# Vidvox/hap

Hardware: AMD Instinct MI355X
Metric: RGBA GB/s + frames/sec, 8K Hap Q encode+decode (higher is better)
Workload: dtype u8; 1 GPU; C4: 7680x4320 0x1, 24 chunks, Snappy, 60-frame stream, device-resident; fragment_index=True, parallelism=single GPU

## Files before the change

hap_amd/csrc/bc_encode.hip:

```cpp
#include <hip/hip_runtime.h>
#include <stdint.h>

#include "bc_encode_core.hpp"
#include "hapgpu_runtime.hpp"

namespace {

using namespace hapbc;

template <int FMT, bool WIDE>
__device__ __forceinline__ void encode_block(const uint8_t *__restrict__ rgba, size_t row_bytes, unsigned blocks_x,
                                             uint8_t *__restrict__ out, uint8_t *__restrict__ out2 = nullptr)
{
    const unsigned by = blockIdx.y, bx = blockIdx.x * 64u + threadIdx.x;
    if (bx >= blocks_x)
        return;
    const size_t id = (size_t)by * blocks_x + bx;
    const uint8_t *src = rgba + (size_t)(4u * by) * row_bytes + 16u * bx;
    unsigned p[16];
#pragma unroll
    for (int r = 0; r < 4; r++) {
        if (WIDE) {
            const uint4 v = *reinterpret_cast<const uint4 *>(src + (size_t)r * row_bytes);
            p[4 * r + 0] = v.x; p[4 * r + 1] = v.y; p[4 * r + 2] = v.z; p[4 * r + 3] = v.w;
        } else {
            const unsigned *q = reinterpret_cast<const unsigned *>(src + (size_t)r * row_bytes);
            p[4 * r + 0] = q[0]; p[4 * r + 1] = q[1]; p[4 * r + 2] = q[2]; p[4 * r + 3] = q[3];
        }
    }
    if (FMT == kFmtRGTC1 || FMT == kFmtDXT1) {
        const uint4 b = block_of<FMT>(p);
        *reinterpret_cast<uint2 *>(out + id * 8u) = make_uint2(b.x, b.y);
    } else {
        *reinterpret_cast<uint4 *>(out + id * 16u) = block_of<FMT == kFmtYCoCgAlpha ? kFmtYCoCg : FMT>(p);
        if (FMT == kFmtYCoCgAlpha) {
            const uint4 a = block_of<kFmtRGTC1>(p);
            *reinterpret_cast<uint2 *>(out2 + id * 8u) = make_uint2(a.x, a.y);
        }
    }
}

template <int FMT, bool WIDE>
__global__ __launch_bounds__(64) void bc_encode_kernel(HapGpuPictureTable t, size_t row_bytes, unsigned blocks_x)
{
    const uint8_t *rgba = (const uint8_t *)picture_address(t, 0);
    uint8_t *out = (uint8_t *)picture_address(t, 1);
    uint8_t *out2 = FMT == kFmtYCoCgAlpha ? (uint8_t *)picture_address(t, 2) : nullptr;
    if (!rgba || !out || (FMT == kFmtYCoCgAlpha && !out2))
        return;
    encode_block<FMT, WIDE>(rgba, row_bytes, blocks_x, out, out2);
}

template <int FMT>
void launch(const HapGpuPictureTable &t, unsigned pictures, size_t row_bytes, unsigned bx, unsigned by, bool wide,
            hipStream_t stream)
{
    const dim3 grid((bx + 63u) / 64u, by, pictures), block(64);
    if (wide)
        hipLaunchKernelGGL((bc_encode_kernel<FMT, true>), grid, block, 0, stream, t, row_bytes, bx);
    else
        hipLaunchKernelGGL((bc_encode_kernel<FMT, false>), grid, block, 0, stream, t, row_bytes, bx);
}

}

extern "C" int hapgpu_k_block_encode(hapgpu_rt *rt, const HapGpuPictureTable *table, unsigned pictures, unsigned width,
                                     unsigned height, size_t row_bytes, unsigned format, int with_alpha, int wide,
                                     unsigned picture_kind)
{
    scoped_timing st(rt, 0);
    const hipStream_t stream = hapgpu_rt_stream(rt);
    const bool half = picture_kind == HAPGPU_PICTURE_RGBA16F, plane = picture_kind == HAPGPU_PICTURE_A8;
    if (picture_kind > HAPGPU_PICTURE_A8 || half != (format == 0x8E8F || format == 0x8E8E) ||
        (plane && (format != 0x8DBB || with_alpha || height / 4u > 65535u)))
        return 1;
    if (!table || !(table->column[0] || table->one[0]) || !(table->column[1] || table->one[1]) ||
        (with_alpha && (format != 0x01 || !(table->column[2] || table->one[2]))) || pictures == 0 || pictures > 65535u ||
        width == 0 || height == 0 || (width & 3u) || (height & 3u) || row_bytes < (size_t)width * HAPGPU_PICTURE_TEXEL_BYTES(picture_kind) ||
        (row_bytes & (half ? 15u : 3u)))
        return 1;
    const HapGpuPictureTable &t = *table;
    const unsigned bx = width / 4u, by = height / 4u;
    switch (format) {
    case 0x83F0: launch<kFmtDXT1>(t, pictures, row_bytes, bx, by, wide != 0, stream); break;
    case 0x83F3: launch<kFmtDXT5>(t, pictures, row_bytes, bx, by, wide != 0, stream); break;
    case 0x01:
        if (with_alpha)
            launch<kFmtYCoCgAlpha>(t, pictures, row_bytes, bx, by, wide != 0, stream);
        else
            launch<kFmtYCoCg>(t, pictures, row_bytes, bx, by, wide != 0, stream);
        break;
    case 0x8DBB:
        if (plane)
            hapgpu_launch_alpha_encode(t, pictures, bx, by, row_bytes, wide != 0, stream);
        else
            launch<kFmtRGTC1>(t, pictures, row_bytes, bx, by, wide != 0, stream);
        break;
    case 0x8E8C: hapgpu_launch_bptc_encode(t, pictures, bx, by, row_bytes, wide != 0, stream); break;
    case 0x8E8F:
    case 0x8E8E: hapgpu_launch_bc6h_encode(t, pictures, format == 0x8E8E, bx, by, row_bytes, stream); break;
    default: return 1;
    }
    return hipGetLastError() == hipSuccess ? 0 : 4;
}
```

hap_amd/csrc/bc_encode_core.hpp:

```cpp
#pragma once
#include <hip/hip_runtime.h>
#include <stdint.h>

namespace hapbc {

constexpr int kFmtDXT1 = 0, kFmtDXT5 = 1, kFmtYCoCg = 2, kFmtRGTC1 = 3;
constexpr int kFmtYCoCgAlpha = 4;

__device__ __forceinline__ int mad24(int a, int b, int c)
{
    int r;
    asm("v_mad_i32_i24 %0, %1, %2, %3" : "=v"(r) : "v"(a), "v"(b), "v"(c));
    return r;
}
template <int K>
__device__ __forceinline__ int mad24k(int a, int c)
{
    int r;
    asm("v_mad_i32_i24 %0, %1, %2, %3" : "=v"(r) : "v"(a), "i"(K), "v"(c));
    return r;
}

__device__ __forceinline__ int quant5(int v) { int t = mad24k<31>(v, 128); return (t + (t >> 8)) >> 8; }
__device__ __forceinline__ int quant6(int v) { int t = mad24k<63>(v, 128); return (t + (t >> 8)) >> 8; }
__device__ __forceinline__ int expand5(int q) { return (q << 3) | (q >> 2); }
__device__ __forceinline__ int expand6(int q) { return (q << 2) | (q >> 4); }


__device__ __forceinline__ unsigned ramp_codes(unsigned w)
{
    return w ^ (~((w >> 1) | (w >> 2)) & 0x249249u);
}

__device__ __forceinline__ uint2 alpha_block(const int (&a)[16])
{
    int lo = a[0], hi = a[0];
#pragma unroll
    for (int i = 1; i < 16; i++) {
        lo = min(lo, a[i]);
        hi = max(hi, a[i]);
    }
    const int a0 = hi, a1 = lo;
    unsigned lo24 = 0, hi24 = 0;
    if (a0 != a1) {
        const int d = a0 - a1;
        unsigned q = (unsigned)(524288.0f * __builtin_amdgcn_rcpf((float)d));
        const int rem = 524288 - (int)__umul24(q, (unsigned)d);
        q += (rem >= d ? 1u : 0u) - (rem < 0 ? 1u : 0u);
        const unsigned m = q + 1u;
        const int neg_m14 = -(int)(14u * m);
        const int start = mad24(a0, (int)(14u * m), (int)__umul24((unsigned)max(d - 6, 0), m)) + (1 << 20);
#pragma unroll
        for (int i = 0; i < 16; i++) {
            const unsigned r1 = (unsigned)mad24(a[i], neg_m14, start) >> 20;
            if (i < 8)
                lo24 = __builtin_amdgcn_alignbit(r1, lo24, 3);
            else
                hi24 = __builtin_amdgcn_alignbit(r1, hi24, 3);
        }
        lo24 = ramp_codes(lo24 >> 8);
        hi24 = ramp_codes(hi24 >> 8);
    }
    const unsigned long long bits = (unsigned long long)lo24 | ((unsigned long long)hi24 << 24);
    const unsigned long long v = (unsigned long long)(unsigned)a0 | ((unsigned long long)(unsigned)a1 << 8) | (bits << 16);
    return make_uint2((unsigned)v, (unsigned)(v >> 32));
}

struct projection {
    unsigned adir;
    unsigned flip;
    int start;
    int top;
    unsigned m24;
};

__device__ __forceinline__ unsigned index_scale(unsigned len2)
{
    unsigned m = (unsigned)(50331648.0f * __builtin_amdgcn_rcpf((float)len2));
    const int rem = (int)(50331648u - m * len2);
    m += (rem >= (int)len2 ? 1u : 0u) - (rem < 0 ? 1u : 0u);
    return m;
}

template <int CHANNELS = 3>
__device__ __forceinline__ projection make_projection(unsigned p0, unsigned p1)
{
    projection pr;
    int dir[CHANNELS];
    unsigned adir = 0, flip = 0;
    int neg = 0, base = 0;
#pragma unroll
    for (int c = 0; c < CHANNELS; c++) {
        const int a = (int)((p0 >> (8 * c)) & 255u), b = (int)((p1 >> (8 * c)) & 255u);
        dir[c] = a - b;
        const int ad = abs(dir[c]);
        adir |= (unsigned)ad << (8 * c);
        flip |= (dir[c] < 0 ? 0xFFu : 0u) << (8 * c);
        neg += dir[c] < 0 ? ad : 0;
        base = mad24(b, dir[c], base);
    }
    const unsigned len2 = __builtin_amdgcn_udot4(adir, adir, 0u, false);
    const unsigned sixth = __umulhi(len2, 0xAAAAAAABu) >> 2;
    pr.adir = adir;
    pr.flip = flip;
    pr.start = (int)sixth - base - 255 * neg;
    pr.top = (int)(len2 + sixth);
    pr.m24 = index_scale(len2);
    return pr;
}

template <bool FLIPPED = false>
__device__ __forceinline__ unsigned project4(const unsigned (&px)[16], const projection &pr)
{
    unsigned pos2 = 0;
#pragma unroll
    for (int i = 0; i < 16; i++) {
        const unsigned q = FLIPPED ? px[i] : px[i] ^ pr.flip;
        const int t = (int)__builtin_amdgcn_udot4(q, pr.adir, (unsigned)pr.start, false);
        const int pos = min(max(__mul24(t, (int)pr.m24) >> 24, 0), 3);
        pos2 = __builtin_amdgcn_alignbit((unsigned)pos, pos2, 2);
    }
    const unsigned hi = pos2 & 0xAAAAAAAAu;
    const unsigned idx = (hi ^ ((pos2 << 1) & 0xAAAAAAAAu)) | ((~hi >> 1) & 0x55555555u);
    return idx;
}

__device__ __forceinline__ unsigned pack3(int a, int b, int c) { return (unsigned)a | ((unsigned)b << 8) | ((unsigned)c << 16); }

__device__ __forceinline__ unsigned expand_565(unsigned c, bool blue)
{
    return pack3(expand5(c >> 11), expand6((c >> 5) & 63), blue ? expand5(c & 31) : 0);
}

__device__ __forceinline__ uint2 colour_block(const unsigned (&px)[16])
{
    int lo[3] = {255, 255, 255}, hi[3] = {0, 0, 0};
#pragma unroll
    for (int i = 0; i < 16; i++) {
#pragma unroll
        for (int c = 0; c < 3; c++) {
            const int v = (int)((px[i] >> (8 * c)) & 255u);
            lo[c] = min(lo[c], v);
            hi[c] = max(hi[c], v);
        }
    }
    int cov_rg = 0, cov_bg = 0;
    const int mr = lo[0] + hi[0], mg = lo[1] + hi[1], mb = lo[2] + hi[2];
#pragma unroll
    for (int i = 0; i < 16; i++) {
        const int dr = 2 * (int)(px[i] & 255u) - mr;
        const int dg = 2 * (int)((px[i] >> 8) & 255u) - mg;
        const int db = 2 * (int)((px[i] >> 16) & 255u) - mb;
        cov_rg = mad24(dr, dg, cov_rg);
        cov_bg = mad24(db, dg, cov_bg);
    }
#pragma unroll
    for (int c = 0; c < 3; c++) {
        const int inset = (hi[c] - lo[c]) >> 4;
        lo[c] += inset;
        hi[c] -= inset;
    }
    const int ar = cov_rg < 0 ? lo[0] : hi[0], br = cov_rg < 0 ? hi[0] : lo[0];
    const int ab = cov_bg < 0 ? lo[2] : hi[2], bb = cov_bg < 0 ? hi[2] : lo[2];
    const unsigned qa = (unsigned)(quant5(ar) << 11 | quant6(hi[1]) << 5 | quant5(ab));
    const unsigned qb = (unsigned)(quant5(br) << 11 | quant6(lo[1]) << 5 | quant5(bb));
    const unsigned c0 = max(qa, qb), c1 = min(qa, qb);
    unsigned idx = 0;
    if (c0 != c1)
        idx = project4(px, make_projection(expand_565(c0, true), expand_565(c1, true)));
    return make_uint2(c0 | (c1 << 16), idx);
}

typedef unsigned short pk_u16 __attribute__((ext_vector_type(2)));
typedef short pk_i16 __attribute__((ext_vector_type(2)));

__device__ __forceinline__ uint2 ycocg_colour_block(const unsigned (&cc)[16])
{
    pk_u16 lo = __builtin_bit_cast(pk_u16, cc[0]), hi = lo;
#pragma unroll
    for (int i = 1; i < 16; i++) {
        const pk_u16 v = __builtin_bit_cast(pk_u16, cc[i]);
        lo = __builtin_elementwise_min(lo, v);
        hi = __builtin_elementwise_max(hi, v);
    }
    int lo_o = lo.x, hi_o = hi.x, lo_g = lo.y, hi_g = hi.y;
    const int m = max(max(128 - lo_o, hi_o - 128), max(128 - lo_g, hi_g - 128));
    const int s = m <= 31 ? 4 : (m <= 63 ? 2 : 1);
    int prod = 0;
    pk_u16 sums = {0, 0};
#pragma unroll
    for (int i = 0; i < 16; i++) {
        int r;
        asm("v_mad_i32_i16 %0, %1, %1, %2 op_sel:[0,1,0,0]" : "=v"(r) : "v"(cc[i]), "v"(prod));
        prod = r;
        sums += __builtin_bit_cast(pk_u16, cc[i]);
    }
    const int mo = lo_o + hi_o, mg = lo_g + hi_g;
    const int cov = 4 * prod - 2 * mg * (int)sums.x - 2 * mo * (int)sums.y + 16 * mo * mg;
    lo_o = (lo_o - 128) * s + 128; hi_o = (hi_o - 128) * s + 128;
    lo_g = (lo_g - 128) * s + 128; hi_g = (hi_g - 128) * s + 128;
    int ins = (hi_o - lo_o) >> 4; lo_o += ins; hi_o -= ins;
    ins = (hi_g - lo_g) >> 4; lo_g += ins; hi_g -= ins;
    const int ag = cov < 0 ? lo_g : hi_g, bg = cov < 0 ? hi_g : lo_g;
    const int qo_a = quant5(hi_o), qo_b = quant5(lo_o), qg_a = quant6(ag), qg_b = quant6(bg);
    const unsigned qa = (unsigned)(qo_a << 11 | qg_a << 5 | (s - 1));
    const unsigned qb = (unsigned)(qo_b << 11 | qg_b << 5 | (s - 1));
    const unsigned c0 = max(qa, qb), c1 = min(qa, qb);
    unsigned idx = 0;
    if (c0 != c1) {
        const bool sw = qa < qb;
        const int eo_a = expand5(qo_a), eo_b = expand5(qo_b), eg_a = expand6(qg_a), eg_b = expand6(qg_b);
        const int d_o = sw ? eo_b - eo_a : eo_a - eo_b, d_g = sw ? eg_b - eg_a : eg_a - eg_b;
        const int p1_o = sw ? eo_a : eo_b, p1_g = sw ? eg_a : eg_b;
        const unsigned len2 = (unsigned)mad24(d_o, d_o, __mul24(d_g, d_g));
        const int sixth = (int)(__umulhi(len2, 0xAAAAAAABu) >> 2);
        const unsigned m24 = index_scale(len2);
        const int centre = 128 - 128 * s;
        const int K = mad24(d_o, centre - p1_o, mad24(d_g, centre - p1_g, sixth));
        const pk_i16 dir2 = {(short)d_o, (short)d_g};
        constexpr int kDotOffset = 1 << 17;
        const unsigned sm = (unsigned)s * m24;
        const unsigned Km = (unsigned)(K - s * kDotOffset) * m24;
        unsigned pos2 = 0;
#pragma unroll
        for (int i = 0; i < 16; i++) {
            unsigned dot;
            asm("v_dot2_i32_i16 %0, %1, %2, %3\n\ts_nop 2" : "=v"(dot) : "v"(cc[i]), "v"(__builtin_bit_cast(unsigned, dir2)), "s"(kDotOffset));
            const int pos = min(max((int)(__umul24(dot, sm) + Km) >> 24, 0), 3);
            pos2 = __builtin_amdgcn_alignbit((unsigned)pos, pos2, 2);
        }
        const unsigned hi = pos2 & 0xAAAAAAAAu;
        idx = (hi ^ ((pos2 << 1) & 0xAAAAAAAAu)) | ((~hi >> 1) & 0x55555555u);
    }
    return make_uint2(c0 | (c1 << 16), idx);
}

template <int FMT>
__device__ __forceinline__ uint4 block_of(const unsigned (&p)[16])
{
    if (FMT == kFmtRGTC1) {
        int a[16];
#pragma unroll
        for (int i = 0; i < 16; i++)
            a[i] = (int)(p[i] >> 24);
        const uint2 ab = alpha_block(a);
        return make_uint4(ab.x, ab.y, 0u, 0u);
    } else if (FMT == kFmtDXT1) {
        unsigned px[16];
#pragma unroll
        for (int i = 0; i < 16; i++)
            px[i] = p[i] & 0x00FFFFFFu;
        const uint2 cb = colour_block(px);
        return make_uint4(cb.x, cb.y, 0u, 0u);
    } else if (FMT == kFmtDXT5) {
        int a[16];
        unsigned px[16];
#pragma unroll
        for (int i = 0; i < 16; i++) {
            a[i] = (int)(p[i] >> 24);
            px[i] = p[i] & 0x00FFFFFFu;
        }
        const uint2 ab = alpha_block(a), cb = colour_block(px);
        return make_uint4(ab.x, ab.y, cb.x, cb.y);
    } else {
        int y[16];
        unsigned cc[16];
#pragma unroll
        for (int i = 0; i < 16; i++) {
            const unsigned q = p[i];
            y[i] = (int)(__builtin_amdgcn_udot4(q, 0x00010201u, 2u, false) >> 2);
            const unsigned co2 = __builtin_amdgcn_udot4(q ^ 0x00FF0000u, 0x00010001u, 2u, false);
            const unsigned cg4 = __builtin_amdgcn_udot4(q ^ 0x00FF00FFu, 0x00010201u, 4u, false);
            const pk_u16 raw = __builtin_bit_cast(pk_u16, co2 | (cg4 << 16)), sh = {1, 2};
            cc[i] = __builtin_bit_cast(unsigned, (pk_u16)(raw >> sh));
        }
        const uint2 ab = alpha_block(y), cb = ycocg_colour_block(cc);
        return make_uint4(ab.x, ab.y, cb.x, cb.y);
    }
}

}
```

hap_amd/csrc/snappy_compress_blocks.hip:

```cpp
#include <hip/hip_runtime.h>
#include <stdint.h>
#include "hapgpu_runtime.hpp"
#include "measurement_guard.h"
#include "bc_encode_core.hpp"

namespace {

constexpr unsigned kFragBytes = 8192u;
constexpr unsigned kSteps = kFragBytes / 1024u;
constexpr unsigned kTableBits = 9u;
constexpr unsigned kDistances = 4u;

template <unsigned LAYOUT> struct unit_layout;
template <> struct unit_layout<4u> {
    static constexpr unsigned block = 16u, code = 4u;
    static constexpr unsigned small32 = 0x11111111u;
    static constexpr unsigned big32 = 0x22222222u;
    static constexpr unsigned four32 = 0xCCCCCCCCu;
    static constexpr unsigned run3_12 = 0xBBBBBBBBu;
    static constexpr unsigned run15_61 = 0x22222222u;
    __device__ static constexpr unsigned fo(unsigned k) { return k == 0u ? 0u : k == 1u ? 2u : k == 2u ? 8u : 12u; }
    __device__ static constexpr unsigned fs(unsigned k) { return k == 0u ? 2u : k == 1u ? 6u : 4u; }
    __device__ static constexpr unsigned cls(unsigned k) { return k == 1u ? 1u : k == 3u ? 3u : 0u; }
};
template <> struct unit_layout<2u> {
    static constexpr unsigned block = 8u, code = 10u;
    static constexpr unsigned small32 = 0u, big32 = 0u, four32 = 0xFFFFFFFFu, run3_12 = 0xFFFFFFFFu, run15_61 = 0u;
    __device__ static constexpr unsigned fo(unsigned k) { return 4u * k; }
    __device__ static constexpr unsigned fs(unsigned) { return 4u; }
    __device__ static constexpr unsigned cls(unsigned k) { return (k & 1u) ? 1u : 0u; }
};
template <> struct unit_layout<8u> {
    static constexpr unsigned block = 16u, code = 12u;
    static constexpr unsigned small32 = 0u, big32 = 0u, four32 = 0xFFFFFFFFu, run3_12 = 0xFFFFFFFFu, run15_61 = 0u;
    __device__ static constexpr unsigned fo(unsigned k) { return 4u * k; }
    __device__ static constexpr unsigned fs(unsigned) { return 4u; }
    __device__ static constexpr unsigned cls(unsigned k) { return k == 1u ? 1u : k == 3u ? 3u : 0u; }
};
template <> struct unit_layout<6u> {
    static constexpr unsigned block = 8u, code = 2u;
    static constexpr unsigned small32 = 0x55555555u, big32 = 0xAAAAAAAAu, four32 = 0u, run3_12 = 0xAAAAAAAAu,
                              run15_61 = 0xAAAAAAAAu;
    __device__ static constexpr unsigned fo(unsigned k) { return k == 0u ? 0u : k == 1u ? 2u : k == 2u ? 8u : 10u; }
    __device__ static constexpr unsigned fs(unsigned k) { return (k & 1u) ? 6u : 2u; }
    __device__ static constexpr unsigned cls(unsigned k) { return (k & 1u) ? 1u : 0u; }
};

typedef const uint8_t __attribute__((address_space(1))) *gsrc_t;
typedef uint8_t __attribute__((address_space(1))) *gdst_t;
struct __attribute__((packed)) pk_u16 { uint16_t v; };
struct __attribute__((packed)) pk_u32 { uint32_t v; };
struct __attribute__((packed)) pk_u64 { uint32_t a, b; };
struct __attribute__((packed)) pk_u128 { uint32_t a, b, c, d; };
__device__ __forceinline__ void put8(gdst_t p, unsigned v) { *p = (uint8_t)v; }
__device__ __forceinline__ void put16(gdst_t p, unsigned v) { reinterpret_cast<pk_u16 __attribute__((address_space(1))) *>(p)->v = (uint16_t)v; }
__device__ __forceinline__ void put32(gdst_t p, unsigned v) { reinterpret_cast<pk_u32 __attribute__((address_space(1))) *>(p)->v = v; }
__device__ __forceinline__ void put64(gdst_t p, uint2 v)
{
    pk_u64 __attribute__((address_space(1))) *q = reinterpret_cast<pk_u64 __attribute__((address_space(1))) *>(p);
    q->a = v.x; q->b = v.y;
}
__device__ __forceinline__ void put128(gdst_t p, uint4 v)
{
    pk_u128 __attribute__((address_space(1))) *q = reinterpret_cast<pk_u128 __attribute__((address_space(1))) *>(p);
    q->a = v.x; q->b = v.y; q->c = v.z; q->d = v.w;
}
__device__ __forceinline__ uint4 get128(gsrc_t p)
{
    const pk_u128 __attribute__((address_space(1))) *q = reinterpret_cast<const pk_u128 __attribute__((address_space(1))) *>(p);
    return make_uint4(q->a, q->b, q->c, q->d);
}
__device__ __forceinline__ uint2 get64(gsrc_t p)
{
    const pk_u64 __attribute__((address_space(1))) *q = reinterpret_cast<const pk_u64 __attribute__((address_space(1))) *>(p);
    return make_uint2(q->a, q->b);
}

__device__ __forceinline__ unsigned rotr(unsigned v, unsigned n) { return __builtin_amdgcn_alignbit(v, v, n); }
__device__ __forceinline__ unsigned bfi(unsigned mask, unsigned a, unsigned b) { return (a & mask) | (b & ~mask); }
__device__ __forceinline__ unsigned popc(unsigned v) { return (unsigned)__builtin_popcount(v); }
__device__ __forceinline__ unsigned nonzero(unsigned v)
{
    unsigned r;
    asm("v_min_u32 %0, 1, %1" : "=v"(r) : "v"(v));
    return r;
}
__device__ __forceinline__ unsigned bit_mask(unsigned v, unsigned bit) { return (unsigned)__builtin_amdgcn_sbfe((int)v, bit, 1u); }

__device__ __forceinline__ int scan_add(int v)
{
    v += __builtin_amdgcn_update_dpp(0, v, 0x111, 0xF, 0xF, false);
    v += __builtin_amdgcn_update_dpp(0, v, 0x112, 0xF, 0xF, false);
    v += __builtin_amdgcn_update_dpp(0, v, 0x114, 0xF, 0xF, false);
    v += __builtin_amdgcn_update_dpp(0, v, 0x118, 0xF, 0xF, false);
    v += __builtin_amdgcn_update_dpp(0, v, 0x142, 0xA, 0xF, false);
    v += __builtin_amdgcn_update_dpp(0, v, 0x143, 0xC, 0xF, false);
    return v;
}

__device__ __forceinline__ unsigned lane_xor4(unsigned v)
{
    int t = __builtin_amdgcn_update_dpp(0, (int)v, 0x104, 0xF, 0x5, false);
    t = __builtin_amdgcn_update_dpp(t, (int)v, 0x114, 0xF, 0xA, false);
    return (unsigned)t;
}
__device__ __forceinline__ unsigned lane_xor2(unsigned v) { return (unsigned)__builtin_amdgcn_update_dpp(0, (int)v, 0x4E, 0xF, 0xF, false); }
__device__ __forceinline__ unsigned lane_xor1(unsigned v) { return (unsigned)__builtin_amdgcn_update_dpp(0, (int)v, 0xB1, 0xF, 0xF, false); }

template <unsigned LAYOUT>
__device__ __forceinline__ unsigned differ_nibble(unsigned acc, const uint4 x, const uint4 y, unsigned d)
{
    const unsigned d0 = x.x ^ y.x, d1 = x.y ^ y.y, d2 = x.z ^ y.z, d3 = x.w ^ y.w;
    unsigned t0, t1, t2, t3;
    if (LAYOUT == 4u) {
        t0 = d0 & 0xFFFFu; t1 = (d0 & 0xFFFF0000u) | d1; t2 = d2; t3 = d3;
    } else if (LAYOUT == 2u || LAYOUT == 8u) {
        t0 = d0; t1 = d1; t2 = d2; t3 = d3;
    } else {
        t0 = d0 & 0xFFFFu; t1 = (d0 & 0xFFFF0000u) | d1; t2 = d2 & 0xFFFFu; t3 = (d2 & 0xFFFF0000u) | d3;
    }
    acc |= nonzero(t0) << (4u * d);
    acc |= nonzero(t1) << (4u * d + 1u);
    acc |= nonzero(t2) << (4u * d + 2u);
    acc |= nonzero(t3) << (4u * d + 3u);
    return acc;
}

template <unsigned LAYOUT>
__device__ __forceinline__ void index_field(const uint4 x, unsigned k, unsigned &lo, unsigned &hi)
{
    if (LAYOUT == 2u || LAYOUT == 8u) {
        lo = k == 1u ? x.y : x.w;
        hi = 0u;
    } else if (k == 1u) {
        lo = __builtin_amdgcn_alignbit(x.y, x.x, 16);
        hi = x.y >> 16;
    } else if (LAYOUT == 4u) {
        lo = x.w;
        hi = 0u;
    } else {
        lo = __builtin_amdgcn_alignbit(x.w, x.z, 16);
        hi = x.w >> 16;
    }
}

__device__ __forceinline__ unsigned table_slot(unsigned lo, unsigned hi, unsigned cls)
{
    const unsigned z = lo ^ rotr(hi, 19) ^ (cls << 29);
    return (z * 0x9E3779B1u) >> (32u - kTableBits);
}

#ifndef SCB_MIN_WAVES
#define SCB_MIN_WAVES 1
#endif
template <unsigned LAYOUT, int FUSED>
__global__ __launch_bounds__(64, SCB_MIN_WAVES) void snappy_compress_blocks_kernel(const HapGpuFrameEnc *__restrict__ frames,
                                                                    uint8_t *__restrict__ slots, unsigned slot_stride,
                                                                    uint32_t *__restrict__ frag_sizes,
                                                                    uint8_t *__restrict__ group_tables)
{
    using UL = unit_layout<LAYOUT>;
    constexpr unsigned B = UL::block;
    __shared__ unsigned long long table[1u << kTableBits];
    __shared__ __attribute__((aligned(16))) uint32_t masks[64u * 8u];
    __shared__ uint32_t bounds[66];

    const unsigned lane = threadIdx.x;
#ifdef PLC_NO_INTERLEAVE
    const unsigned zf = blockIdx.z, x = blockIdx.x;
#else
    const unsigned linear = blockIdx.z * gridDim.x + blockIdx.x;
    const unsigned zf = gridDim.y == 1u ? linear % gridDim.z : blockIdx.z;
    const unsigned x = gridDim.y == 1u ? linear / gridDim.z : blockIdx.x;
#endif
    const HapGpuTexEnc tex = frames[zf].tex[blockIdx.y < 2u ? blockIdx.y : 0u];
    const unsigned tex_count = frames[zf].tex_count;
    if ((blockIdx.y >= tex_count) | (tex.compressor != 1u) | (((tex.reserved >> 16) & 0xFu) != UL::code) |
        (x >= tex.chunk_count * tex.frags_per_chunk) | (tex.src == 0) | (tex.chunk_bytes == 0) |
        (((tex.reserved >> 24) & 7u) != (unsigned)(FUSED + 1)))
        return;
    const unsigned chunk = x / tex.frags_per_chunk, fj = x - chunk * tex.frags_per_chunk;
    const unsigned begin = fj * kFragBytes;
    const unsigned n = min(kFragBytes, tex.chunk_bytes - begin);
    const gsrc_t src = (gsrc_t)(tex.src + (uint64_t)chunk * tex.chunk_bytes + begin);
    const unsigned f = tex.frag_first + x;
    gdst_t out = (gdst_t)((uintptr_t)slots + (size_t)f * slot_stride);
    const bool placed = ((tex.reserved >> 27) & 1u) != 0u && blockIdx.y == 0u;
    const unsigned window = ((tex.reserved >> 8) & 0xFFu) ? ((tex.reserved >> 8) & 0xFFu) * 256u : 0xFFFFFFFFu;
    const bool want_sizes = ((tex.reserved >> 20) & 1u) != 0u && group_tables != nullptr;
    gdst_t table_at = (gdst_t)((uintptr_t)group_tables + (size_t)f * HAP_GROUP_TABLE_BYTES);

    {
        uint4 *t = reinterpret_cast<uint4 *>(table);
#pragma unroll
        for (unsigned i = 0; i < (sizeof(table) / 16u) / 64u; i++)
            t[i * 64u + lane] = make_uint4(0, 0, 0, 0);
    }
    __syncthreads();

    const unsigned keep4 = (lane & 4u) ? 0xFFFF0000u : 0x0000FFFFu;
    const unsigned keep2 = (lane & 2u) ? 0xFF00FF00u : 0x00FF00FFu;
    const unsigned keep1 = (lane & 1u) ? 0xF0F0F0F0u : 0x0F0F0F0Fu;
    const unsigned rot2 = (lane & 2u) ? 8u : 24u;
    const unsigned rot1 = (lane & 1u) ? 4u : 28u;
    const unsigned last = n - (B == 16u ? 16u : 8u);

    constexpr unsigned kSub = 16u / B;
    __shared__ __attribute__((aligned(16))) uint4 ring[FUSED >= 0 ? 68u : 1u];
    const gsrc_t rgba = (gsrc_t)frames[zf].rgba;
    const unsigned row_bytes = frames[zf].rgba_row_bytes, blocks_x = frames[zf].rgba_blocks_x;
    unsigned bx[kSub], by[kSub], first_off = 0u;
#ifdef SCB_PREFETCH
    constexpr bool kPrefetch = SCB_PREFETCH != 0;
#else
    constexpr bool kPrefetch = FUSED != hapbc::kFmtYCoCg;
#endif
    unsigned pix[kPrefetch ? 2 : 1][16];
    auto load_pixels = [&](unsigned (&p)[16], unsigned t) {
        const unsigned sub = t % kSub;
        const bool there = (64u * t + lane + 1u) * B <= n;
        const unsigned at = there ? (4u * by[sub]) * row_bytes + 16u * bx[sub] : first_off;
#pragma unroll
        for (unsigned r = 0; r < 4u; r++) {
            const uint4 v = get128(rgba + (at + r * row_bytes));
            p[4u * r] = v.x; p[4u * r + 1u] = v.y; p[4u * r + 2u] = v.z; p[4u * r + 3u] = v.w;
        }
    };
    auto next_block = [&](unsigned sub) {
        bx[sub] += 64u * kSub;
        while (bx[sub] >= blocks_x) {
            bx[sub] -= blocks_x;
            by[sub] += 1u;
        }
    };
    if (FUSED >= 0) {
        const unsigned first_block = (unsigned)(((uint64_t)chunk * tex.chunk_bytes + begin) / B);
        {
            const unsigned fy = first_block / blocks_x, fx = first_block - fy * blocks_x;
            first_off = (4u * fy) * row_bytes + 16u * fx;
        }
#pragma unroll
        for (unsigned j = 0; j < kSub; j++) {
            const unsigned b = first_block + 64u * j + lane;
            by[j] = b / blocks_x;
            bx[j] = b - by[j] * blocks_x;
        }
        load_pixels(pix[0], 0u);
    }

    constexpr bool kKeepX = !(FUSED >= 0 && B == 8u);
    uint4 X[kKeepX ? kSteps : 1u];
    unsigned HD[kSteps];
#pragma unroll
    for (unsigned s = 0; s < kSteps; s++) {
        const unsigned pos = (64u * s + lane) * 16u;
        if (kKeepX)
            X[s] = make_uint4(0, 0, 0, 0);
        HD[s] = 0u;
        if (64u * s * 16u >= n) {
            masks[64u * s + lane] = 0u;
            continue;
        }
        const unsigned pc = min(pos, last);
        uint4 xs, Y[kDistances];
        if (FUSED >= 0) {
            uint4 made = make_uint4(0, 0, 0, 0);
#pragma unroll
            for (unsigned sub = 0; sub < kSub; sub++) {
                const unsigned t = kSub * s + sub;
                if (!kPrefetch) {
                    if (t > 0u) {
                        if (t >= kSub)
                            next_block(t % kSub);
                        load_pixels(pix[0], t);
                    }
                } else if (t + 1u < kSub * kSteps && 64u * (t + 1u) * B < n) {
                    if (t + 1u >= kSub)
                        next_block((t + 1u) % kSub);
                    load_pixels(pix[(t + 1u) & 1u], t + 1u);
                }
                const uint4 blk = hapbc::block_of<FUSED>(pix[kPrefetch ? t & 1u : 0u]);
                made = blk;
                const unsigned bpos = (64u * t + lane) * B;
                if (B == 16u) {
                    if (bpos + 16u <= n && !placed)
                        put128((gdst_t)(uintptr_t)(src + bpos), blk);
                    ring[4u + lane] = blk;
                } else {
                    if (bpos + 8u <= n)
                        put64((gdst_t)(uintptr_t)(src + bpos), make_uint2(blk.x, blk.y));
                    reinterpret_cast<uint2 *>(ring)[8u + 64u * sub + lane] = make_uint2(blk.x, blk.y);
                }
            }
            __syncthreads();
            const uint8_t *rb = reinterpret_cast<const uint8_t *>(ring) + (4u + lane) * 16u;
            xs = B == 16u ? made : *reinterpret_cast<const uint4 *>(rb);
#pragma unroll
            for (unsigned d = 0; d < kDistances; d++) {
                if (B == 16u) {
                    Y[d] = *reinterpret_cast<const uint4 *>(rb - (d + 1u) * 16u);
                } else {
                    const uint2 ylo = *reinterpret_cast<const uint2 *>(rb - (d + 1u) * 8u), yhi = *reinterpret_cast<const uint2 *>(rb - (d + 1u) * 8u + 8u);
                    Y[d] = make_uint4(ylo.x, ylo.y, yhi.x, yhi.y);
                }
            }
            __syncthreads();
            if (lane >= 60u)
                ring[lane - 60u] = xs;
        } else if (B == 16u) {
            xs = get128(src + pc);
#pragma unroll
            for (unsigned d = 0; d < kDistances; d++) {
                const unsigned back = (d + 1u) * B;
                Y[d] = get128(src + (s == 0u ? max(pc, back) - back : pc - back));
            }
        } else {
            const uint2 lo = get64(src + pc), hi = get64(src + min(pos + 8u, last));
            xs = make_uint4(lo.x, lo.y, hi.x, hi.y);
#pragma unroll
            for (unsigned d = 0; d < kDistances; d++) {
                const unsigned back = (d + 1u) * B;
                if (s == 0u) {
                    const uint2 ylo = get64(src + max(pc, back) - back), yhi = get64(src + max(pc + 8u, back) - back);
                    Y[d] = make_uint4(ylo.x, ylo.y, yhi.x, yhi.y);
                } else {
                    Y[d] = get128(src + pc - back);
                }
            }
        }
        if (kKeepX)
            X[s] = xs;
        unsigned differ = 0;
#pragma unroll
        for (unsigned d = 0; d < kDistances; d++)
            differ = differ_nibble<LAYOUT>(differ, xs, Y[d], d);
        unsigned ok = pos + 16u <= n ? 0xFFFFu : 0u;
        if (B == 8u)
            ok = pos + 16u <= n ? 0xFFFFu : pos + 8u <= n ? 0x3333u : 0u;
        if (s == 0u) {
            if (B == 16u)
                ok &= (1u << (4u * min(lane, 4u))) - 1u;
            else
                ok &= lane == 0u ? 0x000Cu : lane == 1u ? 0x0CFFu : 0xFFFFu;
        }
        unsigned P = ~differ & ok;
        const unsigned eq_fixed = P;
        unsigned slot[2], klo[2], khi[2], valid[2];
        unsigned long long e[2];
#pragma unroll
        for (unsigned i = 0; i < 2u; i++) {
            const unsigned k = 2u * i + 1u;
            unsigned lo, hi;
            index_field<LAYOUT>(xs, k, lo, hi);
            klo[i] = lo;
            khi[i] = hi | (UL::cls(k) << 16);
            slot[i] = table_slot(lo, hi, UL::cls(k));
            valid[i] = (i == 0u ? pos + 8u <= n : pos + 16u <= n) ? 0xFFFFFFFFu : 0u;
            e[i] = table[slot[i]];
        }
        unsigned hd2[2];
#pragma unroll
        for (unsigned i = 0; i < 2u; i++) {
            const unsigned unit = 64u * s + lane;
            const unsigned blk = B == 16u ? unit : 2u * unit + i;
            const unsigned elo = (unsigned)e[i], ehi = (unsigned)(e[i] >> 32);
            const unsigned dist = blk - (ehi >> 18);
            const unsigned miss = (elo ^ klo[i]) | ((ehi & 0x3FFFFu) ^ khi[i]) | ~valid[i];
            const bool hit = (miss == 0u) & (dist * B <= window);
            hd2[i] = hit ? dist : 0u;
            P |= hit ? (dist * B >= 2048u ? 0x220000u : 0x020000u) << (2u * i) : 0u;
            const unsigned enter = valid[i] & ~(0u - ((eq_fixed >> (2u * i + 1u)) & 1u));
            atomicMax(&table[slot[i]], ((unsigned long long)((khi[i] | (blk << 18)) & enter) << 32) | (klo[i] & enter));
        }
        HD[s] = hd2[0] | (hd2[1] << 16);
        P = bfi(keep4, P, rotr(lane_xor4(P), 16));
        P = bfi(keep2, P, rotr(lane_xor2(P), rot2));
        P = bfi(keep1, P, rotr(lane_xor1(P), rot1));
        masks[64u * s + lane] = P;
    }
    __syncthreads();

    {
        uint32_t *hd_tab = reinterpret_cast<uint32_t *>(table);
#pragma unroll
        for (unsigned s = 0; s < kSteps; s++)
            hd_tab[64u * s + lane] = HD[s];
    }
    unsigned counts_and_bytes = 0;
    {
        const uint4 ma = *reinterpret_cast<const uint4 *>(&masks[lane * 8u]);
        const uint4 mb = *reinterpret_cast<const uint4 *>(&masks[lane * 8u + 4u]);
        const unsigned fields_total = (n >> 4) * 4u + ((n & 8u) ? 2u : 0u);
        const unsigned nv = fields_total > 32u * lane ? min(32u, fields_total - 32u * lane) : 0u;
        const unsigned valid = nv >= 32u ? 0xFFFFFFFFu : ((1u << nv) - 1u);
        unsigned E[kDistances] = {ma.x, ma.y, ma.z, ma.w}, A[kDistances] = {0u, 0u, 0u, 0u};
        unsigned U = 0;
#pragma unroll
        for (unsigned d = 0; d < kDistances; d++) {
            E[d] &= ~(UL::small32 & ~(E[d] >> 1) & ~(E[d] << 1));
            U |= E[d];
        }
        unsigned front = U & ~(U << 1);
        while (__builtin_amdgcn_ballot_w64(front != 0u) != 0ull) {
            unsigned taken = 0, ends = 0;
#pragma unroll
            for (unsigned dd = 0; dd < kDistances; dd++) {
#ifdef HAP_BLK_FAR_FIRST
                const unsigned d = kDistances - 1u - dd;
#else
                const unsigned d = dd;
#endif
                const unsigned seeds = front & E[d] & ~taken;
                const unsigned sum = E[d] + seeds;
                A[d] |= (E[d] & ~sum) | seeds;
                ends |= sum & ~E[d];
                taken |= seeds;
            }
            front = ends & U;
        }
        const unsigned cov = A[0] | A[1] | A[2] | A[3];
        unsigned Hm = mb.x & ~cov;
        unsigned L = valid & ~(cov | Hm);
        if (UL::four32 != 0u) {
            const unsigned cpy = cov | Hm;
            const unsigned lone4 = cpy & ~(cpy << 1) & ~(cpy >> 1) & UL::four32 & (L << 1) & (L >> 1);
            L |= lone4;
            Hm &= ~lone4;
#pragma unroll
            for (unsigned d = 0; d < kDistances; d++)
                A[d] &= ~lone4;
        }
        unsigned S = 0;
#pragma unroll
        for (int pass = 0; pass < 2; pass++) {
            S = Hm | (L & ~(L << 1));
#pragma unroll
            for (unsigned d = 0; d < kDistances; d++)
                S |= A[d] & ~(A[d] << 1);
            S &= valid;
            {
                constexpr unsigned FO = LAYOUT == 4u ? 0x0C080200u : (LAYOUT == 2u || LAYOUT == 8u) ? 0x0C080400u : 0x0A080200u;
                const unsigned a = 31u - (unsigned)__builtin_clz((S & 0xFFFFu) | 1u);
                const unsigned b = 17u + (unsigned)__builtin_ctz(((S | ~valid) >> 17) | 0x8000u);
                const unsigned bytes = (b >> 2) * 16u + ((FO >> (8u * (b & 3u))) & 0xFFu) - (a >> 2) * 16u - ((FO >> (8u * (a & 3u))) & 0xFFu);
                const unsigned inside = (valid & ~S & ~L) >> 16;
                S |= (inside & (bytes > 64u ? 1u : 0u)) << 16;
            }
            if (pass == 0 && UL::small32 != 0u) {
                const unsigned lone = UL::small32 & S & (((S | ~valid) >> 1) | 0x80000000u) & ~L & ~Hm & valid;
                L |= lone;
#pragma unroll
                for (unsigned d = 0; d < kDistances; d++)
                    A[d] &= ~lone;
            }
        }
        const unsigned Sx1 = ((S | ~valid) >> 1) | 0x80000000u;
        const unsigned CS = S & ~L;
        const unsigned N1 = ~Sx1;
        const unsigned C3 = (CS & N1 & (N1 >> 1) & ((N1 >> 2) | UL::run3_12)) | (Hm & mb.y);
        const unsigned Cn = L & ~S;
        const unsigned w2 = Cn & (Cn >> 1), w4 = w2 & (w2 >> 2), w8 = w4 & (w4 >> 4);
        const unsigned w12 = w8 & (w4 >> 8), w14 = w12 & (w2 >> 12), w15 = w14 & (Cn >> 14);
        const unsigned LS = S & L & ((w15 >> 1) | ((w14 >> 1) & UL::run15_61));
        const unsigned X3 = C3 | LS;
        const unsigned D0 = A[1] | A[3], D1 = A[2] | A[3];
        const unsigned lit_bytes = 4u * popc(L) - 2u * popc(L & UL::small32) + 2u * popc(L & UL::big32);
        const unsigned total = lit_bytes + popc(S) + popc(CS) + popc(X3);
        const unsigned count = popc(S);
        const unsigned both = (unsigned)scan_add((int)(total | (count << 16)));
        const unsigned incl = both & 0xFFFFu;
        const unsigned base = incl - total;
        *reinterpret_cast<uint4 *>(&masks[lane * 8u]) = make_uint4(S, L, X3, D0);
        *reinterpret_cast<uint4 *>(&masks[lane * 8u + 4u]) = make_uint4(D1, Hm, Sx1, base | (((both >> 16) - count) << 16));
        if (lane == 63u) {
            if (placed) {
                __hip_atomic_store(&frag_sizes[f], incl | HAPGPU_FRAG_PUBLISHED, __ATOMIC_RELAXED, __HIP_MEMORY_SCOPE_AGENT);
            } else {
                frag_sizes[f] = incl;
            }
        }
        counts_and_bytes = both;
        {
            uint8_t *elfield = reinterpret_cast<uint8_t *>(table) + 2048u;
            unsigned left = S, at = (both >> 16) - count, first = 0x80u;
            while (__builtin_amdgcn_ballot_w64(left != 0u) != 0ull) {
                if (left != 0u) {
                    elfield[at] = (uint8_t)(first | (unsigned)__builtin_ctz(left));
                    left &= left - 1u;
                    at += 1u;
                    first = 0u;
                }
            }
        }
    }
    __syncthreads();

    constexpr unsigned kPlacedMaxPolls = 1u << 12;
    if (placed) {
        const unsigned long long *acc = reinterpret_cast<const unsigned long long *>(frames[zf].chunk_acc);
        const uint32_t *mine = frag_sizes + tex.frag_first + chunk * tex.frags_per_chunk;
        unsigned long long sum = 0;
        unsigned in_chunk = 0;
        unsigned tries = 0;
        bool settled = true;
        for (unsigned c0 = 0; c0 < chunk && settled; c0 += 64u) {
            const unsigned c = c0 + lane;
            for (;;) {
                const unsigned long long v = c < chunk ? __hip_atomic_load(&acc[c], __ATOMIC_RELAXED, __HIP_MEMORY_SCOPE_AGENT)
                                                       : (1ull << 32);
                if (__builtin_amdgcn_ballot_w64((unsigned)(v >> 32) == 0u) == 0ull) {
                    sum += v & 0xFFFFFFFFull;
                    settled = __builtin_amdgcn_ballot_w64((unsigned)(v >> 32) != 1u) == 0ull;
                    break;
                }
                if (++tries > kPlacedMaxPolls) {
                    settled = false;
                    break;
                }
                __builtin_amdgcn_s_sleep(16);
            }
        }
        for (unsigned k0 = 0; k0 < fj && settled; k0 += 64u) {
            const unsigned k = k0 + lane;
            for (;;) {
                const unsigned v = k < fj ? __hip_atomic_load(&mine[k], __ATOMIC_RELAXED, __HIP_MEMORY_SCOPE_AGENT) : HAPGPU_FRAG_PUBLISHED;
                if (__builtin_amdgcn_ballot_w64((v & HAPGPU_FRAG_PUBLISHED) == 0u) == 0ull) {
                    in_chunk += v & ~HAPGPU_FRAG_PUBLISHED;
                    break;
                }
                if (++tries > kPlacedMaxPolls) {
                    settled = false;
                    break;
                }
                __builtin_amdgcn_s_sleep(16);
            }
        }
        const unsigned own_bytes = (unsigned)__builtin_amdgcn_readlane((int)counts_and_bytes, 63) & 0xFFFFu;
        if (settled) {
#pragma unroll
            for (int d = 32; d > 0; d >>= 1) {
                sum += __shfl_xor(sum, d);
                in_chunk += __shfl_xor(in_chunk, d);
            }
            if (fj + 1u == tex.frags_per_chunk && lane == 0u)
                __hip_atomic_store(const_cast<unsigned long long *>(&acc[chunk]), (1ull << 32) | (in_chunk + own_bytes), __ATOMIC_RELAXED,
                                   __HIP_MEMORY_SCOPE_AGENT);
            sum += in_chunk;
            const unsigned n_chunks = tex.chunk_count, fpc = tex.frags_per_chunk;
            const bool with_tiles = tex.emit_index && want_sizes;
            const unsigned index_len = tex.emit_index ? 8u + (with_tiles ? 4u + HAP_GROUP_TABLE_BYTES : 4u) * n_chunks * fpc : 0u;
            const unsigned cb = tex.chunk_bytes;
            const unsigned vlen = cb < (1u << 7) ? 1u : cb < (1u << 14) ? 2u : cb < (1u << 21) ? 3u : cb < (1u << 28) ? 4u : 5u;
            const unsigned long long at = frames[zf].dst + frames[zf].outer_header_len + tex.header_len + 4u +
                                          (5u * n_chunks + 8u + index_len) + (unsigned long long)vlen * (chunk + 1u) + sum;
            const unsigned at_lo = (unsigned)__builtin_amdgcn_readfirstlane((int)(unsigned)at);
            const unsigned at_hi = (unsigned)__builtin_amdgcn_readfirstlane((int)(unsigned)(at >> 32));
            out = (gdst_t)(uintptr_t)(((unsigned long long)at_hi << 32) | at_lo);
            if (with_tiles)
                table_at = (gdst_t)(uintptr_t)(frames[zf].dst + frames[zf].outer_header_len + tex.header_len + 8u + n_chunks + 4u +
                                               4u * n_chunks + 8u + 4u * n_chunks * fpc +
                                               (unsigned long long)(chunk * fpc + fj) * HAP_GROUP_TABLE_BYTES);
        } else if (lane == 0u) {
            __hip_atomic_fetch_or(const_cast<uint32_t *>(&frames[zf].reserved), 1u, __ATOMIC_RELAXED, __HIP_MEMORY_SCOPE_AGENT);
            if (fj + 1u == tex.frags_per_chunk)
                __hip_atomic_store(const_cast<unsigned long long *>(&acc[chunk]), 2ull << 32, __ATOMIC_RELAXED, __HIP_MEMORY_SCOPE_AGENT);
        }
    }

    const unsigned j4 = 4u * (lane & 7u);
    const unsigned below = (1u << j4) - 1u;
#pragma unroll
    for (unsigned s = 0; s < kSteps; s++) {
        if (64u * s * 16u >= n)
            continue;
        const unsigned hh = 8u * s + (lane >> 3);
        const uint4 ma = *reinterpret_cast<const uint4 *>(&masks[hh * 8u]);
        const unsigned S = ma.x, L = ma.y, X3 = ma.z, CS = S & ~L;
        unsigned off = (masks[hh * 8u + 7u] & 0xFFFFu) + 4u * popc(L & below) + 2u * popc(L & UL::big32 & below) -
                       2u * popc(L & UL::small32 & below) + popc(S & below) + popc(CS & below) + popc(X3 & below);
        const unsigned sj = S >> j4, lj = L >> j4, xj = X3 >> j4;
        uint4 xs;
        if (kKeepX) {
            xs = X[s];
        } else {
            const unsigned pos = (64u * s + lane) * 16u;
            const uint2 lo = get64(src + min(pos, last)), hi = get64(src + min(pos + 8u, last));
            xs = make_uint4(lo.x, lo.y, hi.x, hi.y);
        }
        constexpr bool kDwords = LAYOUT == 2u || LAYOUT == 8u;
        const unsigned fw[4] = {xs.x, kDwords ? xs.y : xs.x >> 16, xs.z, LAYOUT == 4u ? xs.w : kDwords ? xs.w : xs.z >> 16};
#pragma unroll
        for (unsigned k = 0; k < 4u; k++) {
            const unsigned is_s = bit_mask(sj, k), is_l = bit_mask(lj, k), x3 = bit_mask(xj, k);
            off += is_s & ((is_l & 1u) + (~is_l & 2u) + (x3 & 1u));
            if (is_l) {
                if (UL::fs(k) == 2u) {
                    put16(out + off, fw[k]);
                } else if (UL::fs(k) == 4u) {
                    put32(out + off, fw[k]);
                } else {
                    put16(out + off, fw[k]);
                    put32(out + off + 2, k == 1u ? xs.y : xs.w);
                }
            }
            off += is_l & UL::fs(k);
        }
    }

    {
        const unsigned both = counts_and_bytes;
        const unsigned stream_bytes = (unsigned)__builtin_amdgcn_readlane((int)both, 63) & 0xFFFFu;
        const unsigned elements = (unsigned)__builtin_amdgcn_readlane((int)both, 63) >> 16;
        const unsigned G = (elements + 63u) >> 6;
        const unsigned inv = (1u << 20) / G + 1u;
        const uint32_t *hd_tab = reinterpret_cast<const uint32_t *>(table);
        {
            bounds[lane] = stream_bytes | (n << 16);
            if (lane < 2u)
                bounds[64u + lane] = stream_bytes | (n << 16);
        }
        __syncthreads();
        constexpr unsigned FO = LAYOUT == 4u ? 0x0C080200u : (LAYOUT == 2u || LAYOUT == 8u) ? 0x0C080400u : 0x0A080200u;
        const uint8_t *elfield = reinterpret_cast<const uint8_t *>(table) + 2048u;
        unsigned carry = 0;
#pragma unroll 1
        for (unsigned e0 = 0; e0 < elements; e0 += 64u) {
            const unsigned e = e0 + lane;
            const unsigned info = e < elements ? elfield[e] : 0u;
            const unsigned begun = (unsigned)scan_add((int)(info >> 7)) + carry;
            carry = (unsigned)__builtin_amdgcn_readlane((int)begun, 63);
            if (e < elements) {
                const unsigned h = begun - 1u, q = info & 31u;
                const uint4 ma = *reinterpret_cast<const uint4 *>(&masks[h * 8u]);
                const uint4 mb = *reinterpret_cast<const uint4 *>(&masks[h * 8u + 4u]);
                const unsigned S = ma.x, L = ma.y, X3 = ma.z, D0 = ma.w, D1 = mb.x, Hm = mb.y, Sx1 = mb.z, CS = S & ~L;
                const unsigned under = (1u << q) - 1u;
                const unsigned off = (mb.w & 0xFFFFu) + 4u * popc(L & under) + 2u * popc(L & UL::big32 & under) -
                                     2u * popc(L & UL::small32 & under) + popc(S & under) + popc(CS & under) + popc(X3 & under);
                const unsigned qn = q + 1u + (unsigned)__builtin_ctz(Sx1 >> q);
                const unsigned len = (qn >> 2) * 16u + ((FO >> (8u * (qn & 3u))) & 0xFFu) - (q >> 2) * 16u - ((FO >> (8u * (q & 3u))) & 0xFFu);
                const bool is_l = ((L >> q) & 1u) != 0u, x3 = ((X3 >> q) & 1u) != 0u;
                unsigned dist = 1u + ((D0 >> q) & 1u) + 2u * ((D1 >> q) & 1u);
                if ((Hm >> q) & 1u)
                    dist = (hd_tab[h * 8u + (q >> 2)] >> (8u * (q & 2u))) & 0xFFFFu;
                const unsigned offset = dist * B;
                const unsigned lit = x3 ? 0xF0u | ((len - 1u) << 8) : (len - 1u) << 2;
                const unsigned cpy = x3 ? 2u | ((len - 1u) << 2) | (offset << 8)
                                        : 1u | ((len - 4u) << 2) | ((offset >> 8) << 5) | ((offset & 0xFFu) << 8);
                const unsigned v = is_l ? lit : cpy;
                if (is_l && !x3)
                    put8(out + off, v);
                else
                    put16(out + off, v);
                if (!is_l && x3)
                    put8(out + off + 2, v >> 16);
                const unsigned m = (e * inv) >> 20;
                if (m * G == e)
                    bounds[m] = off | ((h * 128u + (q >> 2) * 16u + ((FO >> (8u * (q & 3u))) & 0xFFu)) << 16);
            }
        }
        __syncthreads();
        if (want_sizes) {
            const unsigned lo = bounds[lane], hi = bounds[lane + 1u];
            const unsigned entry = ((hi & 0xFFFFu) - (lo & 0xFFFFu)) | (((hi >> 16) - (lo >> 16)) << 12);
            const gdst_t at = table_at + lane * 3u;
            put16(at, entry);
            put8(at + 2, entry >> 16);
            if (lane == 0u) {
                put16(table_at + 192, elements);
                put16(table_at + 194, 0u);
            }
        }
    }
}

}

int hapgpu_snappy_compress_blocks(const HapGpuFrameEnc *frames, unsigned frame_count, unsigned max_frags_per_texture,
                                  unsigned textures, void *slots, unsigned slot_stride, uint32_t *frag_sizes,
                                  uint8_t *group_tables, unsigned layouts, unsigned fused, hipStream_t stream)
{
    if (frame_count == 0 || max_frags_per_texture == 0 || (layouts | fused) == 0)
        return 0;
    const dim3 grid(max_frags_per_texture, textures, frame_count), block(64);
#define HAP_LAUNCH_BLOCKS(L, F)                                                                                                  \
    hipLaunchKernelGGL((snappy_compress_blocks_kernel<L, F>), grid, block, 0, stream, frames, (uint8_t *)slots, slot_stride,    \
                       frag_sizes, group_tables)
    if (fused & 1u)
        HAP_LAUNCH_BLOCKS(4u, hapbc::kFmtYCoCg);
#ifndef SCB_ONLY_FUSED_YCOCG
    if (fused & 2u)
        HAP_LAUNCH_BLOCKS(4u, hapbc::kFmtDXT5);
    if (fused & 12u)
        return 1;
    if (layouts & 1u)
        HAP_LAUNCH_BLOCKS(4u, -1);
    if (layouts & 2u)
        HAP_LAUNCH_BLOCKS(2u, -1);
    if (layouts & 4u)
        HAP_LAUNCH_BLOCKS(6u, -1);
    if (layouts & 8u)
        HAP_LAUNCH_BLOCKS(8u, -1);
#endif
#undef HAP_LAUNCH_BLOCKS
    return hipGetLastError() == hipSuccess ? 0 : 4;
}
```

Baseline: 2487 GB/s.

## Compute YCoCg colour transform with MFMA int8 matrix ops instead of per-pixel dot4

Replaces the per-pixel udot4 YCoCg conversion with a 4x4x4 int8 MFMA, where each lane supplies its row of the Y/Co/Cg weight matrix and pixels are biased to signed bytes. The per-thread early return in the standalone encode kernel becomes clamped indices plus guarded stores, so all lanes stay active for the cross-lane MFMA. Launch bounds for the fused YCoCg Snappy kernel and the encode kernel change, and the fused kernel's initial block-coordinate division is replaced by a wraparound loop. This moves colour math onto the matrix units but adds MFMA latency and a lane-dependent weight setup, which could affect register pressure and occupancy.

```diff
diff --git a/hap_amd/csrc/bc_encode.hip b/hap_amd/csrc/bc_encode.hip
--- a/hap_amd/csrc/bc_encode.hip
+++ b/hap_amd/csrc/bc_encode.hip
@@ -12,9 +12,10 @@
 __device__ __forceinline__ void encode_block(const uint8_t *__restrict__ rgba, size_t row_bytes, unsigned blocks_x,
                                              uint8_t *__restrict__ out, uint8_t *__restrict__ out2 = nullptr)
 {
-    const unsigned by = blockIdx.y, bx = blockIdx.x * 64u + threadIdx.x;
-    if (bx >= blocks_x)
-        return;
+    const unsigned by = blockIdx.y, lane_bx = blockIdx.x * 64u + threadIdx.x;
+    const bool there = lane_bx < blocks_x;
+    const ycocg_matrix ym = make_ycocg_matrix();
+    const unsigned bx = min(lane_bx, blocks_x - 1u);
     const size_t id = (size_t)by * blocks_x + bx;
     const uint8_t *src = rgba + (size_t)(4u * by) * row_bytes + 16u * bx;
     unsigned p[16];
@@ -29,19 +30,23 @@
         }
     }
     if (FMT == kFmtRGTC1 || FMT == kFmtDXT1) {
-        const uint4 b = block_of<FMT>(p);
-        *reinterpret_cast<uint2 *>(out + id * 8u) = make_uint2(b.x, b.y);
+        const uint4 b = block_of<FMT>(p, ym);
+        if (there)
+            *reinterpret_cast<uint2 *>(out + id * 8u) = make_uint2(b.x, b.y);
     } else {
-        *reinterpret_cast<uint4 *>(out + id * 16u) = block_of<FMT == kFmtYCoCgAlpha ? kFmtYCoCg : FMT>(p);
+        const uint4 b = block_of<FMT == kFmtYCoCgAlpha ? kFmtYCoCg : FMT>(p, ym);
+        if (there)
+            *reinterpret_cast<uint4 *>(out + id * 16u) = b;
         if (FMT == kFmtYCoCgAlpha) {
-            const uint4 a = block_of<kFmtRGTC1>(p);
-            *reinterpret_cast<uint2 *>(out2 + id * 8u) = make_uint2(a.x, a.y);
+            const uint4 a = block_of<kFmtRGTC1>(p, ym);
+            if (there)
+                *reinterpret_cast<uint2 *>(out2 + id * 8u) = make_uint2(a.x, a.y);
         }
     }
 }
 
 template <int FMT, bool WIDE>
-__global__ __launch_bounds__(64) void bc_encode_kernel(HapGpuPictureTable t, size_t row_bytes, unsigned blocks_x)
+__global__ __launch_bounds__(64, 2) void bc_encode_kernel(HapGpuPictureTable t, size_t row_bytes, unsigned blocks_x)
 {
     const uint8_t *rgba = (const uint8_t *)picture_address(t, 0);
     uint8_t *out = (uint8_t *)picture_address(t, 1);
diff --git a/hap_amd/csrc/bc_encode_core.hpp b/hap_amd/csrc/bc_encode_core.hpp
--- a/hap_amd/csrc/bc_encode_core.hpp
+++ b/hap_amd/csrc/bc_encode_core.hpp
@@ -235,8 +235,67 @@
     return make_uint2(c0 | (c1 << 16), idx);
 }
 
+#ifndef HAPBC_YCOCG_MFMA
+#define HAPBC_YCOCG_MFMA 1
+#endif
+#ifndef HAPBC_YCOCG_GROUP
+#define HAPBC_YCOCG_GROUP 16
+#endif
+typedef int v4i32 __attribute__((ext_vector_type(4)));
+constexpr unsigned kYWeights = 0x00010201u, kCoWeights = 0x00FF0001u, kCgWeights = 0x00FF02FFu;
+constexpr int kYBias = 514, kCoBias = 257, kCgBias = 514;
+
+struct ycocg_matrix {
+    int weights;
+    v4i32 bias;
+};
+__device__ __forceinline__ ycocg_matrix make_ycocg_matrix()
+{
+    const unsigned row = __builtin_amdgcn_mbcnt_hi(~0u, __builtin_amdgcn_mbcnt_lo(~0u, 0u)) & 3u;
+    ycocg_matrix m;
+    m.weights = (int)(row == 0u ? kYWeights : row == 1u ? kCoWeights : row == 2u ? kCgWeights : 0u);
+    m.bias = v4i32{kYBias, kCoBias, kCgBias, 0};
+    return m;
+}
+
+__device__ __forceinline__ void ycocg_transform(const unsigned (&p)[16], const ycocg_matrix &m, int (&y)[16], unsigned (&cc)[16])
+{
+    const pk_u16 sh = {1, 2};
+#if HAPBC_YCOCG_MFMA
+#pragma unroll
+    for (int g = 0; g < 16; g += HAPBC_YCOCG_GROUP) {
+        v4i32 d[HAPBC_YCOCG_GROUP];
+#pragma unroll
+        for (int i = 0; i < HAPBC_YCOCG_GROUP; i++)
+            d[i] = __builtin_amdgcn_mfma_i32_4x4x4i8(m.weights, (int)(p[g + i] ^ 0x80808080u), m.bias, 0, 0, 0);
+#pragma unroll
+        for (int i = 0; i < HAPBC_YCOCG_GROUP; i++) {
+            y[g + i] = d[i].x >> 2;
+            const pk_u16 raw = __builtin_bit_cast(pk_u16, (unsigned)d[i].y | ((unsigned)d[i].z << 16));
+            cc[g + i] = __builtin_bit_cast(unsigned, (pk_u16)(raw >> sh));
+        }
+#if HAPBC_YCOCG_GROUP < 16
+        __builtin_amdgcn_sched_barrier(0);
+#endif
+    }
+#else
+    const unsigned wy = kYWeights, wo = kCoWeights, wg = kCgWeights;
+#pragma unroll
+    for (int i = 0; i < 16; i++) {
+        const unsigned q = p[i] ^ 0x80808080u;
+        int y4;
+        unsigned co2, cg4;
+        asm("v_dot4_i32_i8 %0, %3, %4, %7\n\tv_dot4_i32_i8 %1, %3, %5, %8\n\tv_dot4_i32_i8 %2, %3, %6, %7\n\ts_nop 2"
+            : "=&v"(y4), "=&v"(co2), "=&v"(cg4) : "v"(q), "v"(wy), "v"(wo), "v"(wg), "s"(kYBias), "s"(kCoBias));
+        y[i] = y4 >> 2;
+        const pk_u16 raw = __builtin_bit_cast(pk_u16, co2 | (cg4 << 16));
+        cc[i] = __builtin_bit_cast(unsigned, (pk_u16)(raw >> sh));
+    }
+#endif
+}
+
 template <int FMT>
-__device__ __forceinline__ uint4 block_of(const unsigned (&p)[16])
+__device__ __forceinline__ uint4 block_of(const unsigned (&p)[16], const ycocg_matrix &ym)
 {
     if (FMT == kFmtRGTC1) {
         int a[16];
@@ -265,15 +324,7 @@
     } else {
         int y[16];
         unsigned cc[16];
-#pragma unroll
-        for (int i = 0; i < 16; i++) {
-            const unsigned q = p[i];
-            y[i] = (int)(__builtin_amdgcn_udot4(q, 0x00010201u, 2u, false) >> 2);
-            const unsigned co2 = __builtin_amdgcn_udot4(q ^ 0x00FF0000u, 0x00010001u, 2u, false);
-            const unsigned cg4 = __builtin_amdgcn_udot4(q ^ 0x00FF00FFu, 0x00010201u, 4u, false);
-            const pk_u16 raw = __builtin_bit_cast(pk_u16, co2 | (cg4 << 16)), sh = {1, 2};
-            cc[i] = __builtin_bit_cast(unsigned, (pk_u16)(raw >> sh));
-        }
+        ycocg_transform(p, ym, y, cc);
         const uint2 ab = alpha_block(y), cb = ycocg_colour_block(cc);
         return make_uint4(ab.x, ab.y, cb.x, cb.y);
     }
diff --git a/hap_amd/csrc/snappy_compress_blocks.hip b/hap_amd/csrc/snappy_compress_blocks.hip
--- a/hap_amd/csrc/snappy_compress_blocks.hip
+++ b/hap_amd/csrc/snappy_compress_blocks.hip
@@ -153,8 +153,11 @@
 #ifndef SCB_MIN_WAVES
 #define SCB_MIN_WAVES 1
 #endif
+#ifndef SCB_YCOCG_WAVES
+#define SCB_YCOCG_WAVES 5
+#endif
 template <unsigned LAYOUT, int FUSED>
-__global__ __launch_bounds__(64, SCB_MIN_WAVES) void snappy_compress_blocks_kernel(const HapGpuFrameEnc *__restrict__ frames,
+__global__ __launch_bounds__(64, (FUSED == hapbc::kFmtYCoCg && HAPBC_YCOCG_MFMA) ? SCB_YCOCG_WAVES : SCB_MIN_WAVES) void snappy_compress_blocks_kernel(const HapGpuFrameEnc *__restrict__ frames,
                                                                     uint8_t *__restrict__ slots, unsigned slot_stride,
                                                                     uint32_t *__restrict__ frag_sizes,
                                                                     uint8_t *__restrict__ group_tables)
@@ -210,6 +213,7 @@
     const gsrc_t rgba = (gsrc_t)frames[zf].rgba;
     const unsigned row_bytes = frames[zf].rgba_row_bytes, blocks_x = frames[zf].rgba_blocks_x;
     unsigned bx[kSub], by[kSub], first_off = 0u;
+    const hapbc::ycocg_matrix ym = hapbc::make_ycocg_matrix();
 #ifdef SCB_PREFETCH
     constexpr bool kPrefetch = SCB_PREFETCH != 0;
 #else
@@ -235,15 +239,16 @@
     };
     if (FUSED >= 0) {
         const unsigned first_block = (unsigned)(((uint64_t)chunk * tex.chunk_bytes + begin) / B);
-        {
-            const unsigned fy = first_block / blocks_x, fx = first_block - fy * blocks_x;
-            first_off = (4u * fy) * row_bytes + 16u * fx;
-        }
+        const unsigned fy = first_block / blocks_x, fx = first_block - fy * blocks_x;
+        first_off = (4u * fy) * row_bytes + 16u * fx;
 #pragma unroll
         for (unsigned j = 0; j < kSub; j++) {
-            const unsigned b = first_block + 64u * j + lane;
-            by[j] = b / blocks_x;
-            bx[j] = b - by[j] * blocks_x;
+            bx[j] = fx + 64u * j + lane;
+            by[j] = fy;
+            while (bx[j] >= blocks_x) {
+                bx[j] -= blocks_x;
+                by[j] += 1u;
+            }
         }
         load_pixels(pix[0], 0u);
     }
@@ -279,7 +284,7 @@
                         next_block((t + 1u) % kSub);
                     load_pixels(pix[(t + 1u) & 1u], t + 1u);
                 }
-                const uint4 blk = hapbc::block_of<FUSED>(pix[kPrefetch ? t & 1u : 0u]);
+                const uint4 blk = hapbc::block_of<FUSED>(pix[kPrefetch ? t & 1u : 0u], ym);
                 made = blk;
                 const unsigned bpos = (64u * t + lane) * B;
                 if (B == 16u) {
```

Result: slower. 2367 GB/s (-4.8%).
